# titus-leistner/mmlf

Hardware: AMD Instinct MI355X
Metric: 96x96 EPI patches/sec fwd+bwd, bs=512 (higher is better)
Workload: dtype f32 via 2 x f16 operand split (22 significant bits per operand, locally scaled; 3 MFMA passes, f32 accumulate)

## Files before the change

mmlf_amd/csrc/build.py:

```python
import os
import subprocess
import sys

HERE = os.path.dirname(os.path.abspath(__file__))
SOURCES = ['conv.hip', 'wgrad.hip', 'elementwise.hip']
LIB = os.path.join(HERE, 'libmmlf_hip.so')
HIPCC = os.environ.get('HIPCC', '/opt/rocm/bin/hipcc')
FLAGS = ['-O3', '--offload-arch=gfx950', '-fPIC', '-std=c++17', '-Wall', '-Wno-unused-function', '-ffp-contract=off']


def stale():
    if not os.path.exists(LIB):
        return True
    t = os.path.getmtime(LIB)
    deps = SOURCES + ['common.h', 'conv_device.h', 'build.py', os.path.join('..', '..', 'include', 'mmlf_hip.h')]
    return any(os.path.getmtime(os.path.join(HERE, d)) > t for d in deps)


def source_revision():
    root = os.path.dirname(os.path.dirname(HERE))
    try:
        rev = subprocess.check_output(['git', '-C', root, 'rev-parse', '--short=12', 'HEAD'], stderr=subprocess.DEVNULL).decode().strip()
        dirty = subprocess.call(['git', '-C', root, 'diff', '--quiet', 'HEAD', '--', 'mmlf_amd/csrc', 'include'],
                                stderr=subprocess.DEVNULL) != 0
        return rev + ('+' if dirty else '')
    except (OSError, subprocess.CalledProcessError):
        return 'unknown'


HASHED = SOURCES + ['common.h', 'conv_device.h', os.path.join('..', '..', 'include', 'mmlf_hip.h')]


def source_hash():
    import hashlib
    h = hashlib.sha1()
    for d in HASHED:
        with open(os.path.join(HERE, d), 'rb') as f:
            h.update(f.read())
    return h.hexdigest()[:12]


def build(force=False, verbose=True, extra_flags=(), lib=None):
    if lib is None and not extra_flags and not force and not stale():
        return LIB
    lib = lib or LIB
    tag = '' if lib == LIB else '.' + os.path.basename(lib).replace('.so', '')
    flags = [*FLAGS, f'-DMMLF_GIT_HASH="{source_revision()}"', f'-DMMLF_SRC_HASH="{source_hash()}"', *extra_flags]
    objs, jobs = [], []
    for src in SOURCES:
        obj = os.path.join(os.path.dirname(lib), src.replace('.hip', tag + '.o'))
        cmd = [HIPCC, *flags, '-c', os.path.join(HERE, src), '-o', obj]
        if verbose:
            print(' '.join(cmd), flush=True)
        jobs.append((cmd, subprocess.Popen(cmd)))
        objs.append(obj)
    failed = [cmd for cmd, job in jobs if job.wait() != 0]
    if failed:
        raise subprocess.CalledProcessError(1, failed[0])
    cmd = [HIPCC, '--offload-arch=gfx950', '-shared', '-fPIC', *objs, '-o', lib]
    if verbose:
        print(' '.join(cmd), flush=True)
    subprocess.check_call(cmd)
    return lib


if __name__ == '__main__':
    if '--source-hash' in sys.argv:
        print(source_hash())
    elif '--source-revision' in sys.argv:
        print(source_revision())
    else:
        build(force='--force' in sys.argv)
```

mmlf_amd/csrc/wgrad.hip:

```cpp
#include "conv_device.h"

#ifdef MMLF_BOUNDS_DEBUG
int mmlf_oob_counts_wgrad(unsigned long long *host8, int reset)
{
    if (hipMemcpyFromSymbol(host8, HIP_SYMBOL(g_mmlf_oob), sizeof(unsigned long long) * 8) != hipSuccess) return 1;
    if (reset) {
        const unsigned long long z[8] = {};
        if (hipMemcpyToSymbol(HIP_SYMBOL(g_mmlf_oob), z, sizeof(z)) != hipSuccess) return 1;
    }
    return 0;
}
#endif

struct WgradArgs {
    const float *in;
    const float *g;
    float *part;
    long long NQpad;
    int cs_in, cin, cs_g, g_shift, P, nsplit, nslice, chunks_per_split, nchunks;
    int g_cols;
    const float *in_amax, *g_amax;
    const float *chunk_scales;
    long long in_bytes, g_bytes, part_floats;
};

__device__ __forceinline__ bool wgrad_block_map(const WgradArgs &a, int &slice, int &split)
{
    const int b = blockIdx.x, x = b & 7, j = b >> 3;
    const int reg = (a.nsplit >> 3) * a.nslice;
    if (j < reg) {
        slice = j % a.nslice;
        split = (j / a.nslice) * 8 + x;
        return true;
    }
    const int left = (a.nsplit & 7) * a.nslice, per = (left + 7) >> 3;
    const int m = x * per + (j - reg);
    slice = m % a.nslice;
    split = (a.nsplit & ~7) + m / a.nslice;
    return m < left;
}

static inline unsigned wgrad_grid_blocks(int nslice, int nsplit)
{
    return 8u * (unsigned)((nsplit >> 3) * nslice + ((nsplit & 7) * nslice + 7) / 8);
}

#define WG_KQ 32

template <int KS>
struct WgradF32Shape {
    static constexpr int WAVES = KS == 2 ? 4 : 3;
    static constexpr int SEGS = KS == 2 ? 2 : 1;
    static constexpr int BPS = KS / SEGS;
    static constexpr int ROWS = WG_KQ + KS - 1;
    static constexpr int A_FL = SEGS * ROWS * 32;
    static constexpr size_t lds_bytes(int nt) { return (A_FL + WG_KQ * nt * 32) * sizeof(float); }
};

template <int KS, int NT>
__device__ __forceinline__ void wgrad_f32_taps(const WgradArgs &a)
{
    using S = WgradF32Shape<KS>;
    constexpr int TAPS = KS * KS, THREADS = 64 * S::WAVES, SEGS = S::SEGS, BPS = S::BPS, ROWS = S::ROWS, A_FL = S::A_FL;
    constexpr int NP = NT * 32;
    constexpr int A_F4 = A_FL / 4;
    constexpr int NA = (A_F4 + THREADS - 1) / THREADS;
    constexpr int G_F4 = WG_KQ * NP / 4;
    constexpr int NG = (G_F4 + THREADS - 1) / THREADS;
    static_assert(KS == 3 || G_F4 % THREADS == 0, "2x2: the gradient tile is a whole number of staging rounds (no guard)");
    extern __shared__ __attribute__((aligned(16))) char smem[];
    float *As = reinterpret_cast<float *>(smem);
    float *Gs = As + A_FL;

    const int tid = threadIdx.x;
    const int lane = tid & 63, wv = tid >> 6;
    const int i = lane & 31, kh = lane >> 5;
    int sd, split;
    if (!wgrad_block_map(a, sd, split)) return;
    const int slice = sd / BPS, dy = sd - BPS * slice;
    const int ci0 = slice * 32;
    int c_begin = split * a.chunks_per_split;
    int c_end = c_begin + a.chunks_per_split;
    if (c_end > a.nchunks) c_end = a.nchunks;

    f32x16 acc[NT];
#pragma unroll
    for (int nt = 0; nt < NT; ++nt)
#pragma unroll
        for (int r = 0; r < 16; ++r) acc[nt][r] = 0.f;

    float4 ra[NA], rg[NG];
    auto gload = [&](int c) {
        const long long Qc = (long long)c * WG_KQ + (long long)dy * a.P;
#pragma unroll
        for (int j = 0; j < NA; ++j) {
            const int idx = tid + THREADS * j;
            float4 v = make_float4(0.f, 0.f, 0.f, 0.f);
            if (idx < A_F4) {
                const int row = idx >> 3, f = idx & 7;
                const int seg = SEGS > 1 && row >= ROWS, pix = row - ROWS * seg;
                const int ch = ci0 + 4 * f;
                if (ch < a.cs_in)
                    v = *reinterpret_cast<const float4 *>(a.in + (size_t)(Qc + seg * a.P + pix) * a.cs_in + ch);
            }
            ra[j] = v;
        }
        const long long Qg = (long long)c * WG_KQ + a.g_shift;
#pragma unroll
        for (int j = 0; j < NG; ++j) {
            const int idx = tid + THREADS * j;
            float4 v = make_float4(0.f, 0.f, 0.f, 0.f);
            if (KS == 2 || idx < G_F4) {
                const int row = idx / (NP / 4), f = idx - row * (NP / 4);
                if (4 * f < a.g_cols) v = *reinterpret_cast<const float4 *>(a.g + (size_t)(Qg + row) * a.cs_g + 4 * f);
            }
            rg[j] = v;
        }
    };
    auto lstore = [&]() {
#pragma unroll
        for (int j = 0; j < NA; ++j) {
            const int idx = tid + THREADS * j;
            if (idx < A_F4) {
                float4 v = ra[j];
                const int ch = ci0 + 4 * (idx & 7);
                if (ch == a.cin) v.x = 1.f;
                if (ch + 1 == a.cin) v.y = 1.f;
                if (ch + 2 == a.cin) v.z = 1.f;
                if (ch + 3 == a.cin) v.w = 1.f;
                reinterpret_cast<float4 *>(As)[idx] = v;
            }
        }
#pragma unroll
        for (int j = 0; j < NG; ++j) {
            const int idx = tid + THREADS * j;
            if (KS == 2 || idx < G_F4) reinterpret_cast<float4 *>(Gs)[idx] = rg[j];
        }
    };

    const int seg = KS == 2 ? wv >> 1 : 0, dx = KS == 2 ? wv & 1 : wv;
    if (c_begin < c_end) {
        gload(c_begin);
        for (int c = c_begin; c < c_end; ++c) {
            lstore();
            __syncthreads();
            if (c + 1 < c_end) gload(c + 1);
            const float *ap = As + (seg * ROWS + dx + kh) * 32 + i;
            const float *gp = Gs + kh * NP + i;
#pragma unroll
            for (int s = 0; s < WG_KQ / 2; ++s) {
                const float av = ap[2 * s * 32];
#pragma unroll
                for (int nt = 0; nt < NT; ++nt) {
                    const float bv = gp[2 * s * NP + 32 * nt];
                    acc[nt] = __builtin_amdgcn_mfma_f32_32x32x2f32(av, bv, acc[nt], 0, 0, 0);
                }
            }
            __syncthreads();
        }
    }
    const int CIP = a.nslice / BPS * 32;
    float *pp = a.part + ((size_t)(split * TAPS + KS * (dy + seg) + dx) * CIP + ci0) * NP;
#pragma unroll
    for (int nt = 0; nt < NT; ++nt)
#pragma unroll
        for (int r = 0; r < 16; ++r) {
            const int row = (r & 3) + 8 * (r >> 2) + 4 * kh;
            pp[(size_t)row * NP + 32 * nt + i] = acc[nt][r];
        }
}

template <int NT>
__global__ __launch_bounds__(256, 2) void wgrad4tap_kernel(WgradArgs a)
{
    wgrad_f32_taps<2, NT>(a);
}

template <int NT>
__global__ __launch_bounds__(192, 2) void wgrad9tap_kernel(WgradArgs a)
{
    wgrad_f32_taps<3, NT>(a);
}

typedef short s16x4 __attribute__((ext_vector_type(4)));
typedef __attribute__((address_space(3))) s16x4 lds_s16x4_t;

__device__ __forceinline__ bf16x8 tr_frag(const char *lds_row0, int row_stride_bytes)
{
    const s16x4 lo = __builtin_amdgcn_ds_read_tr16_b64_v4i16((lds_s16x4_t *)(lds_row0));
    const s16x4 hi = __builtin_amdgcn_ds_read_tr16_b64_v4i16((lds_s16x4_t *)(lds_row0 + 4 * row_stride_bytes));
    return __builtin_shufflevector(lo, hi, 0, 1, 2, 3, 4, 5, 6, 7);
}

__device__ __forceinline__ void split_store4(float4 v, char *p0, int plane_stride_bytes)
{
    unsigned h0, m0, l0, h1, m1, l1;
    split3_pair(v.x, v.y, h0, m0, l0);
    split3_pair(v.z, v.w, h1, m1, l1);
    *reinterpret_cast<uint2 *>(p0) = make_uint2(h0, h1);
    *reinterpret_cast<uint2 *>(p0 + plane_stride_bytes) = make_uint2(m0, m1);
    *reinterpret_cast<uint2 *>(p0 + 2 * plane_stride_bytes) = make_uint2(l0, l1);
}

template <int PL>
__device__ __forceinline__ void split_store4_pl(float4 v, float scale, char *p0, int plane_stride_bytes)
{
    if constexpr (PL == 3) {
        split_store4(v, p0, plane_stride_bytes);
    } else {
        unsigned h0, l0, h1, l1;
        split2_pair_f16<true>(v.x, v.y, scale, h0, l0);
        split2_pair_f16<true>(v.z, v.w, scale, h1, l1);
        *reinterpret_cast<uint2 *>(p0) = make_uint2(h0, h1);
        *reinterpret_cast<uint2 *>(p0 + plane_stride_bytes) = make_uint2(l0, l1);
    }
}
template <int PL>
__device__ __forceinline__ f32x4 mfma16_pl(bf16x8 x, bf16x8 y, f32x4 c)
{
    if constexpr (PL == 3) return __builtin_amdgcn_mfma_f32_16x16x32_bf16(x, y, c, 0, 0, 0);
    else return __builtin_amdgcn_mfma_f32_16x16x32_f16(__builtin_bit_cast(f16x8, x), __builtin_bit_cast(f16x8, y), c, 0, 0, 0);
}
template <int PL> __device__ __forceinline__ constexpr int term_a(int t)
{
    return PL == 3 ? (t == 0 ? 2 : t == 1 ? 0 : t <= 3 ? 1 : 0) : (t == 0 ? 1 : 0);
}
template <int PL> __device__ __forceinline__ constexpr int term_b(int t)
{
    return PL == 3 ? (t == 0 ? 0 : t == 1 ? 2 : t == 2 ? 1 : t == 3 ? 0 : t == 4 ? 1 : 0) : (t == 1 ? 1 : 0);
}
struct WgradScales { float inv_sa, inv_sg; };
template <int PL> __device__ __forceinline__ WgradScales wgrad_scales(const WgradArgs &a)
{
    WgradScales s = {1.f, 1.f};
    if constexpr (PL == 2) {
        s.inv_sa = a.chunk_scales[2 * (size_t)a.nchunks];
        s.inv_sg = a.chunk_scales[2 * (size_t)a.nchunks + 1];
    }
    return s;
}
template <int PL> __device__ __forceinline__ void wgrad_chunk_scale(const WgradArgs &a, int c, float &sa, float &sg)
{
    if constexpr (PL == 2) {
        const float2 v = *reinterpret_cast<const float2 *>(a.chunk_scales + 2 * (size_t)c);
        sa = __uint_as_float(__builtin_amdgcn_readfirstlane(__float_as_uint(v.x)));
        sg = __uint_as_float(__builtin_amdgcn_readfirstlane(__float_as_uint(v.y)));
    } else {
        sa = 1.f; sg = 1.f;
    }
}
struct ChunkScaleArgs {
    const float *in_amax, *g_amax;
    float *out;
    long long NQ;
    int nchunks, P, g_shift, nrows;
    Magic divP;
};
__device__ __forceinline__ int pow2_exponent(float p) { return (int)(__float_as_uint(p) >> 23) - 127; }
__global__ __launch_bounds__(256) void wgrad_chunk_scales_kernel(ChunkScaleArgs a)
{
    const int c = blockIdx.x * 256 + threadIdx.x;
    const float sA = pow2_scale_for(mmlf_amax_tensor_max(a.in_amax)), sG = pow2_scale_for(mmlf_amax_tensor_max(a.g_amax));
    if (c == 0) {
        a.out[2 * (size_t)a.nchunks] = 1.f / sA;
        a.out[2 * (size_t)a.nchunks + 1] = 1.f / sG;
    }
    if (c >= a.nchunks) return;
    const long long q0 = (long long)c * WG_KQ;
    int x = 0;
    if (q0 < a.NQ) {
        const long long ql = q0 + WG_KQ - 1;
        const unsigned r0 = fastdiv((unsigned)q0, a.divP);
        unsigned r1 = fastdiv((unsigned)(ql + a.P + 1), a.divP);
        if (r1 >= (unsigned)a.nrows) r1 = a.nrows - 1;
        float ma = 0.f, mg = 0.f;
        for (unsigned r = r0; r <= r1; ++r) ma = fmaxf(ma, a.in_amax[MMLF_AMAX_HEAD + r]);
        const unsigned g0 = fastdiv((unsigned)(q0 + a.g_shift), a.divP);
        unsigned g1 = fastdiv((unsigned)(ql + a.g_shift), a.divP);
        if (g1 >= (unsigned)a.nrows) g1 = a.nrows - 1;
        for (unsigned r = g0; r <= g1; ++r) mg = fmaxf(mg, a.g_amax[MMLF_AMAX_HEAD + r]);
        const int u = ma > 0.f ? pow2_exponent(pow2_scale_for(ma)) - pow2_exponent(sA) : 60;
        const int v = mg > 0.f ? pow2_exponent(pow2_scale_for(mg)) - pow2_exponent(sG) : 60;
        const int uu = u < 0 ? 0 : u, vv = v < 0 ? 0 : v;
        x = (uu - vv) >> 1;
        x = x > 15 ? 15 : (x < -24 ? -24 : x);
    }
    a.out[2 * (size_t)c] = sA * exp2f((float)x);
    a.out[2 * (size_t)c + 1] = sG * exp2f((float)-x);
}

template <int MB, int NB, int PL>
__global__ __launch_bounds__(256, 2) void wgrad4tap_x6n_kernel(WgradArgs a)
{
    constexpr int ROWA = 32 * (MB | 1), ROWG = 32 * (NB | 1);
    constexpr int A_PLANE = 34 * ROWA;
    constexpr int A_BYTES = 2 * PL * A_PLANE;
    constexpr int NTERM = PL == 3 ? 6 : 3;
    const WgradScales sc = wgrad_scales<PL>(a);
    constexpr int G_PLANE = WG_KQ * ROWG;
    constexpr int FA = 4 * MB, FG = 4 * NB;
    constexpr int NA = (66 * FA + 255) / 256, NG = (WG_KQ * FG + 255) / 256;
    constexpr bool HOLD_G = NB <= 5;
    extern __shared__ __attribute__((aligned(16))) char smem[];
    char *As = smem;
    char *Gs = smem + A_BYTES;

    const int tid = threadIdx.x;
    const int lane = tid & 63, t = tid >> 6;
    const int r16 = lane & 15, q4 = lane >> 4;
    int slice, split;
    if (!wgrad_block_map(a, slice, split)) return;
    const int ci0 = slice * 16 * MB;
    int c_begin = split * a.chunks_per_split;
    int c_end = c_begin + a.chunks_per_split;
    if (c_end > a.nchunks) c_end = a.nchunks;

    f32x4 acc[MB][NB];
#pragma unroll
    for (int mb = 0; mb < MB; ++mb)
#pragma unroll
        for (int nb = 0; nb < NB; ++nb)
#pragma unroll
            for (int r = 0; r < 4; ++r) acc[mb][nb][r] = 0.f;

    float4 ra[NA], rg[NG];
#define WN_GLOAD(c)                                                                                         \
    do {                                                                                                    \
        const long long Qc = (long long)(c) * WG_KQ;                                                        \
        _Pragma("unroll") for (int j = 0; j < NA; ++j) {                                                    \
            const int idx = min(tid + 256 * j, 66 * FA - 1);                                                \
            const int row = idx / FA, f = idx - row * FA;                                                   \
            const int seg = row >= 33, pix = row - 33 * seg;                                                \
            const int ch = min(ci0 + 4 * f, a.cs_in - 4);                                                   \
            MMLF_OOB(OOB_WG_IN, ((Qc + seg * a.P + pix) * a.cs_in + ch + 4) * 4ll > a.in_bytes);            \
            ra[j] = *reinterpret_cast<const float4 *>(a.in + (size_t)(Qc + seg * a.P + pix) * a.cs_in + ch); \
        }                                                                                                   \
        _Pragma("unroll") for (int j = 0; j < NG; ++j) {                                                    \
            const int idx = min(tid + 256 * j, WG_KQ * FG - 1);                                             \
            const int row = idx / FG, f = idx - row * FG;                                                   \
            const int gc = min(4 * f, a.g_cols - 4);                                                        \
            MMLF_OOB(OOB_WG_G, ((Qc + a.g_shift + row) * a.cs_g + gc + 4) * 4ll > a.g_bytes);               \
            rg[j] = *reinterpret_cast<const float4 *>(a.g + (size_t)(Qc + a.g_shift + row) * a.cs_g + gc);  \
        }                                                                                                   \
    } while (0)
#define WN_LSTORE()                                                                                         \
    do {                                                                                                    \
        _Pragma("unroll") for (int j = 0; j < NA; ++j) {                                                    \
            const int idx = min(tid + 256 * j, 66 * FA - 1);                                                \
            const int row = idx / FA, f = idx - row * FA;                                                   \
            const int seg = row >= 33, pix = row - 33 * seg;                                                \
            float4 v = ra[j];                \
            const int ch = ci0 + 4 * f;      \
            if (ch == a.cin) v.x = sc.inv_sa;                                        \
            if (ch + 1 == a.cin) v.y = sc.inv_sa;                                                           \
            if (ch + 2 == a.cin) v.z = sc.inv_sa;                                                           \
            if (ch + 3 == a.cin) v.w = sc.inv_sa;                                                           \
            split_store4_pl<PL>(v, st_sa, As + seg * PL * A_PLANE + pix * ROWA + 8 * f, A_PLANE);           \
        }                                                                                                   \
        _Pragma("unroll") for (int j = 0; j < NG; ++j) {                                                    \
            const int idx = min(tid + 256 * j, WG_KQ * FG - 1);                                             \
            const int row = idx / FG, f = idx - row * FG;                                                   \
            split_store4_pl<PL>(rg[j], st_sg, Gs + row * ROWG + 8 * f, G_PLANE);                            \
        }                                                                                                   \
    } while (0)
    const int tq = (lane & 15) >> 2, tp = lane & 3;
    const char *a_lane = As + (t >> 1) * PL * A_PLANE + ((t & 1) + 4 * q4 + tq) * ROWA + 8 * tp;
    const char *g_lane = Gs + (4 * q4 + tq) * ROWG + 8 * tp;

    float st_sa = 1.f, st_sg = 1.f;
    if (c_begin < c_end) {
        WN_GLOAD(c_begin);
        for (int c = c_begin; c < c_end; ++c) {
            wgrad_chunk_scale<PL>(a, c, st_sa, st_sg);
            WN_LSTORE();
            __syncthreads();
            if (c + 1 < c_end) WN_GLOAD(c + 1);
            if constexpr (HOLD_G) {
                bf16x8 gf[NB][PL];
#pragma unroll
                for (int nb = 0; nb < NB; ++nb)
#pragma unroll
                    for (int pl = 0; pl < PL; ++pl) gf[nb][pl] = tr_frag(g_lane + pl * G_PLANE + 32 * nb, 4 * ROWG);
#pragma unroll
                for (int mb = 0; mb < MB; ++mb) {
                    bf16x8 af[PL];
#pragma unroll
                    for (int pl = 0; pl < PL; ++pl) af[pl] = tr_frag(a_lane + pl * A_PLANE + 32 * mb, 4 * ROWA);
#pragma unroll
                    for (int term = 0; term < NTERM; ++term)
#pragma unroll
                        for (int nb = 0; nb < NB; ++nb)
                            acc[mb][nb] = mfma16_pl<PL>(af[term_a<PL>(term)], gf[nb][term_b<PL>(term)], acc[mb][nb]);
                }
            } else {
                bf16x8 af[MB][PL];
#pragma unroll
                for (int mb = 0; mb < MB; ++mb)
#pragma unroll
                    for (int pl = 0; pl < PL; ++pl) af[mb][pl] = tr_frag(a_lane + pl * A_PLANE + 32 * mb, 4 * ROWA);
#pragma unroll
                for (int nb = 0; nb < NB; ++nb) {
                    bf16x8 gf[PL];
#pragma unroll
                    for (int pl = 0; pl < PL; ++pl) gf[pl] = tr_frag(g_lane + pl * G_PLANE + 32 * nb, 4 * ROWG);
#pragma unroll
                    for (int term = 0; term < NTERM; ++term)
#pragma unroll
                        for (int mb = 0; mb < MB; ++mb)
                            acc[mb][nb] = mfma16_pl<PL>(af[mb][term_a<PL>(term)], gf[term_b<PL>(term)], acc[mb][nb]);
                }
            }
            __syncthreads();
        }
    }
#undef WN_GLOAD
#undef WN_LSTORE
    constexpr int NP = 16 * NB;
    const int CIP = a.nslice * 16 * MB;
    float *pp = a.part + ((size_t)(split * 4 + t) * CIP + ci0) * NP;
#pragma unroll
    for (int mb = 0; mb < MB; ++mb)
#pragma unroll
        for (int nb = 0; nb < NB; ++nb)
#pragma unroll
            for (int r = 0; r < 4; ++r) {
                const int row = 16 * mb + 4 * q4 + r;
                const float un = (ci0 + row == a.cin ? 1.f : sc.inv_sa) * sc.inv_sg;
                MMLF_OOB(OOB_WG_PART, (long long)(pp - a.part) + (long long)row * NP + 16 * nb + r16 >= a.part_floats);
                pp[(size_t)row * NP + 16 * nb + r16] = acc[mb][nb][r] * un;
            }
}

template <int MB, int NBH, int PL>
__global__ __launch_bounds__(512, 2) void wgrad4tap_x6w_kernel(WgradArgs a)
{
    constexpr int NB = 2 * NBH;
    const WgradScales sc = wgrad_scales<PL>(a);
    constexpr int ROWA = 32 * (MB | 1), ROWG = 32 * (NB | 1);
    constexpr int A_PLANE = 34 * ROWA;
    constexpr int A_BYTES = 2 * PL * A_PLANE;
    constexpr int G_PLANE = WG_KQ * ROWG;
    constexpr int BUF_BYTES = A_BYTES + PL * G_PLANE;
    constexpr int FA = 4 * MB, FG = 4 * NB;
    constexpr int NA = (66 * FA + 511) / 512, NG = (WG_KQ * FG + 511) / 512;
    static_assert(2 * BUF_BYTES <= 160 * 1024, "LDS");
    extern __shared__ __attribute__((aligned(16))) char smem[];

    const int tid = threadIdx.x;
    const int lane = tid & 63;
    const int w = __builtin_amdgcn_readfirstlane(tid >> 6);
    const int t = w & 3, h = w >> 2;
    const int r16 = lane & 15, q4 = lane >> 4;
    int slice, split;
    if (!wgrad_block_map(a, slice, split)) return;
    const int ci0 = slice * 16 * MB;
    const int c_begin = split * a.chunks_per_split;
    int c_end = c_begin + a.chunks_per_split;
    if (c_end > a.nchunks) c_end = a.nchunks;

    f32x4 acc[MB][NBH];
#pragma unroll
    for (int mb = 0; mb < MB; ++mb)
#pragma unroll
        for (int nb = 0; nb < NBH; ++nb)
#pragma unroll
            for (int r = 0; r < 4; ++r) acc[mb][nb][r] = 0.f;

    float4 ra[NA], rg[NG];

    unsigned ga_off[NA], gg_off[NG];
    int la_off[NA], lg_off[NG], a_ch[NA];
#pragma unroll
    for (int j = 0; j < NA; ++j) {
        const int idx = min(tid + 512 * j, 66 * FA - 1);
        const int row = idx / FA, f = idx - row * FA;
        const int seg = row >= 33, pix = row - 33 * seg;
        a_ch[j] = ci0 + 4 * f;
        ga_off[j] = (unsigned)((seg * a.P + pix) * a.cs_in + min(ci0 + 4 * f, a.cs_in - 4)) * 4u;
        la_off[j] = seg * PL * A_PLANE + pix * ROWA + 8 * f;
    }
#pragma unroll
    for (int j = 0; j < NG; ++j) {
        const int idx = min(tid + 512 * j, WG_KQ * FG - 1);
        const int row = idx / FG, f = idx - row * FG;
        gg_off[j] = (unsigned)((a.g_shift + row) * a.cs_g + min(4 * f, a.g_cols - 4)) * 4u;
        lg_off[j] = A_BYTES + row * ROWG + 8 * f;
    }
    const char *const in_b = reinterpret_cast<const char *>(a.in), *const g_b = reinterpret_cast<const char *>(a.g);
#define WW_GLOAD_A(j, c)                                                                                    \
    do {                                                                                                    \
        const long long cb_ = (long long)(c) * WG_KQ * a.cs_in * 4;                         \
        MMLF_OOB(OOB_WG_IN, cb_ + ga_off[j] + 16 > a.in_bytes);                                             \
         \
         \
        const __amdgpu_buffer_rsrc_t rs_ = __builtin_amdgcn_make_buffer_rsrc(                               \
            const_cast<char *>(in_b + cb_), 0, mmlf_records_left(a.in_bytes, cb_), MMLF_BUF_FLAGS);         \
        ra[j] = __builtin_bit_cast(float4, __builtin_amdgcn_raw_buffer_load_b128(rs_, ga_off[j], 0, 0));    \
    } while (0)
#define WW_GLOAD_G(j, c)                                                                                    \
    do {                                                                                                    \
        const long long cb_ = (long long)(c) * WG_KQ * a.cs_g * 4;                                          \
        MMLF_OOB(OOB_WG_G, cb_ + gg_off[j] + 16 > a.g_bytes);                                               \
        const __amdgpu_buffer_rsrc_t rs_ = __builtin_amdgcn_make_buffer_rsrc(                               \
            const_cast<char *>(g_b + cb_), 0, mmlf_records_left(a.g_bytes, cb_), MMLF_BUF_FLAGS);           \
        rg[j] = __builtin_bit_cast(float4, __builtin_amdgcn_raw_buffer_load_b128(rs_, gg_off[j], 0, 0));    \
    } while (0)
#define WW_GLOAD(c)                                                                                         \
    do {                                                                                                    \
        _Pragma("unroll") for (int j = 0; j < NA; ++j) WW_GLOAD_A(j, c);                                    \
        _Pragma("unroll") for (int j = 0; j < NG; ++j) WW_GLOAD_G(j, c);                                    \
    } while (0)
#define WW_STORE_A(j, dst)                                                                                  \
    do {                                                                                                    \
        float4 v = ra[j];                                                    \
        const int ch = a_ch[j];                                                                             \
        v.x = ch == a.cin ? sc.inv_sa : v.x;                                         \
        v.y = ch + 1 == a.cin ? sc.inv_sa : v.y;                                                            \
        v.z = ch + 2 == a.cin ? sc.inv_sa : v.z;                                                            \
        v.w = ch + 3 == a.cin ? sc.inv_sa : v.w;                                                            \
        split_store4_pl<PL>(v, st_sa, (dst) + la_off[j], A_PLANE);                                          \
    } while (0)
#define WW_STORE_G(j, dst) split_store4_pl<PL>(rg[j], st_sg, (dst) + lg_off[j], G_PLANE)

    const int tq = (lane & 15) >> 2, tp = lane & 3;
    const int a_off = (t >> 1) * PL * A_PLANE + ((t & 1) + 4 * q4 + tq) * ROWA + 8 * tp;
    const int g_off = A_BYTES + (4 * q4 + tq) * ROWG + 8 * tp + 32 * NBH * h;

    float st_sa = 1.f, st_sg = 1.f;
    if (c_begin < c_end) {
        WW_GLOAD(c_begin);
        wgrad_chunk_scale<PL>(a, c_begin, st_sa, st_sg);
#pragma unroll
        for (int j = 0; j < NA; ++j) WW_STORE_A(j, smem);
#pragma unroll
        for (int j = 0; j < NG; ++j) WW_STORE_G(j, smem);
        if (c_begin + 1 < c_end) WW_GLOAD(c_begin + 1);
        __syncthreads();
        int buf = 0;
        constexpr bool EARLY = PL == 2 && NBH % 3 == 0 && NA + NG <= NBH - 2 && MB >= 2;
        bf16x8 af[MB][PL], gfr[3][PL], afp[2][PL];
        if constexpr (EARLY) {
            const char *cur0 = smem;
#pragma unroll
            for (int g0 = 0; g0 < 2; ++g0)
#pragma unroll
                for (int pl = 0; pl < PL; ++pl) gfr[g0][pl] = tr_frag(cur0 + g_off + pl * G_PLANE + 32 * g0, 4 * ROWG);
#pragma unroll
            for (int mb = 0; mb < 2; ++mb)
#pragma unroll
                for (int pl = 0; pl < PL; ++pl) af[mb][pl] = tr_frag(cur0 + a_off + pl * A_PLANE + 32 * mb, 4 * ROWA);
        }
#define WW_TERM(gf, pa, pb)                                                                                  \
    _Pragma("unroll") for (int mb = 0; mb < MB; ++mb)                                                        \
        acc[mb][nb] = mfma16_pl<PL>(af[mb][pa], gf[pb], acc[mb][nb])
#define WW_CHUNK(STAGE, RELOAD)                                                                              \
    do {                                                                                                     \
        const char *cur = smem + buf * BUF_BYTES;                                                            \
        char *nxt = smem + (buf ^ 1) * BUF_BYTES;                                                            \
        if (!EARLY) {                                                                                        \
            _Pragma("unroll") for (int g0 = 0; g0 < 2; ++g0)                                                 \
                _Pragma("unroll") for (int pl = 0; pl < PL; ++pl)                                             \
                    gfr[g0][pl] = tr_frag(cur + g_off + pl * G_PLANE + 32 * g0, 4 * ROWG);                   \
        }                                                                                                    \
        _Pragma("unroll") for (int mb = EARLY ? 2 : 0; mb < MB; ++mb)                                        \
            _Pragma("unroll") for (int pl = 0; pl < PL; ++pl)                                                 \
                af[mb][pl] = tr_frag(cur + a_off + pl * A_PLANE + 32 * mb, 4 * ROWA);                        \
        _Pragma("unroll") for (int nb = 0; nb < NBH; ++nb) {                                                 \
            if (EARLY && (STAGE) && nb == NBH - 2) {                                                         \
                asm volatile("s_waitcnt lgkmcnt(0)" ::: "memory");    \
                __syncthreads();                                                                             \
                _Pragma("unroll") for (int mb = 0; mb < 2; ++mb)                                             \
                    _Pragma("unroll") for (int pl = 0; pl < PL; ++pl)                                         \
                        afp[mb][pl] = tr_frag(nxt + a_off + pl * A_PLANE + 32 * mb, 4 * ROWA);               \
            }                                                                                                \
            if (nb + 2 < NBH) {                                                                              \
                _Pragma("unroll") for (int pl = 0; pl < PL; ++pl)                                             \
                    gfr[(nb + 2) % 3][pl] = tr_frag(cur + g_off + pl * G_PLANE + 32 * (nb + 2), 4 * ROWG);   \
            } else if (EARLY && (STAGE)) {                                                                   \
                _Pragma("unroll") for (int pl = 0; pl < PL; ++pl)                                             \
                    gfr[(nb + 2) % 3][pl] = tr_frag(nxt + g_off + pl * G_PLANE + 32 * (nb + 2 - NBH), 4 * ROWG); \
            }                                                                                                \
            if (STAGE) {                                                                                     \
                if (nb < NA) {                                                                               \
                    WW_STORE_A(nb < NA ? nb : 0, nxt);                                                       \
                    if (RELOAD) WW_GLOAD_A(nb < NA ? nb : 0, c + 2);                                         \
                } else if (nb - NA < NG) {                                                                   \
                    WW_STORE_G(nb - NA < NG ? nb - NA : 0, nxt);                                             \
                    if (RELOAD) WW_GLOAD_G(nb - NA < NG ? nb - NA : 0, c + 2);                               \
                }                                                                                            \
            }                                                                                                \
            _Pragma("unroll") for (int term = 0; term < (PL == 3 ? 6 : 3); ++term)                           \
                WW_TERM(gfr[nb % 3], term_a<PL>(term), term_b<PL>(term));                                    \
        }                                                                                                    \
        if (EARLY && (STAGE)) {                                                                              \
            _Pragma("unroll") for (int mb = 0; mb < 2; ++mb)                                                 \
                _Pragma("unroll") for (int pl = 0; pl < PL; ++pl) af[mb][pl] = afp[mb][pl];                   \
        }                                                                                                    \
    } while (0)
        static_assert(NA + NG <= NBH, "one staging piece per column block");
        for (int c = c_begin; c + 1 < c_end; ++c) {
            wgrad_chunk_scale<PL>(a, c + 1, st_sa, st_sg);
            const bool reload = c + 2 < c_end;
            WW_CHUNK(true, reload);
            if constexpr (!EARLY) __syncthreads();
            buf ^= 1;
        }
        {
            const int c = c_end - 1;
            (void)c;
            WW_CHUNK(false, false);
        }
#undef WW_CHUNK
#undef WW_TERM
    }
#undef WW_GLOAD
#undef WW_GLOAD_A
#undef WW_GLOAD_G
#undef WW_STORE_A
#undef WW_STORE_G
    constexpr int NP = 16 * NB;
    const int CIP = a.nslice * 16 * MB;
    float *pp = a.part + ((size_t)(split * 4 + t) * CIP + ci0) * NP + 16 * NBH * h;
#pragma unroll
    for (int mb = 0; mb < MB; ++mb)
#pragma unroll
        for (int nb = 0; nb < NBH; ++nb)
#pragma unroll
            for (int r = 0; r < 4; ++r) {
                const int row = 16 * mb + 4 * q4 + r;
                const float un = (ci0 + row == a.cin ? 1.f : sc.inv_sa) * sc.inv_sg;
                MMLF_OOB(OOB_WG_PART, (long long)(pp - a.part) + (long long)row * NP + 16 * nb + r16 >= a.part_floats);
                pp[(size_t)row * NP + 16 * nb + r16] = acc[mb][nb][r] * un;
            }
}

template <int NTAP>
__global__ void wgrad_reduce_kernel(const float *__restrict__ part, float *__restrict__ gw, float *__restrict__ gb,
                                     int Cin, int Cout, int CIP, int NP, int nsplit, int variant, int accumulate)
{
    const int total = NTAP * (Cin + 1) * Cout;
    const int idx = blockIdx.x * blockDim.x + threadIdx.x;
    if (idx >= total) return;
    const int co = idx % Cout;
    int r = idx / Cout;
    const int ci = r % (Cin + 1);
    const int t = r / (Cin + 1);
    if (ci == Cin && (t != 0 || gb == nullptr)) return;
    const float *pp = part + ((size_t)t * CIP + ci) * NP + co;
    const size_t stride = (size_t)NTAP * CIP * NP;
    constexpr int U = 16;
    double acc[U];
#pragma unroll
    for (int u = 0; u < U; ++u) acc[u] = 0.0;
    int sp = 0;
    for (; sp + U <= nsplit; sp += U) {
        float v[U];
#pragma unroll
        for (int u = 0; u < U; ++u) v[u] = pp[(size_t)(sp + u) * stride];
#pragma unroll
        for (int u = 0; u < U; ++u) acc[u] += v[u];
    }
    for (; sp < nsplit; ++sp) acc[0] += pp[(size_t)sp * stride];
#pragma unroll
    for (int h = U / 2; h > 0; h >>= 1)
#pragma unroll
        for (int u = 0; u < h; ++u) acc[u] += acc[u + h];
    const double s = acc[0];
    if (ci == Cin) {
        gb[co] = accumulate ? gb[co] + (float)s : (float)s;
    } else {
        const size_t o = ((size_t)co * Cin + ci) * NTAP + master_tap<(NTAP == 4 ? 2 : 3)>(t, variant);
        gw[o] = accumulate ? gw[o] + (float)s : (float)s;
    }
}

__global__ __launch_bounds__(256) void wgrad_reduce_wave_kernel(const float *__restrict__ part, float *__restrict__ gw,
                                                                float *__restrict__ gb, int Cin, int Cout, int CIP, int NP,
                                                                int nsplit, int variant, int accumulate)
{
    const int total = 4 * (Cin + 1) * Cout;
    const int idx = blockIdx.x * 4 + (threadIdx.x >> 6), lane = threadIdx.x & 63;
    if (idx >= total) return;
    const int co = idx % Cout;
    int r = idx / Cout;
    const int ci = r % (Cin + 1);
    const int t = r / (Cin + 1);
    if (ci == Cin && (t != 0 || gb == nullptr)) return;
    const float *pp = part + ((size_t)t * CIP + ci) * NP + co;
    const size_t stride = (size_t)4 * CIP * NP;
    double acc = 0.0;
    for (int sp = lane; sp < nsplit; sp += 64) acc += pp[(size_t)sp * stride];
#pragma unroll
    for (int o = 32; o > 0; o >>= 1) acc += __shfl_xor(acc, o);
    if (lane) return;
    if (ci == Cin) {
        gb[co] = accumulate ? gb[co] + (float)acc : (float)acc;
    } else {
        const size_t o = ((size_t)co * Cin + ci) * 4 + master_tap<2>(t, variant);
        gw[o] = accumulate ? gw[o] + (float)acc : (float)acc;
    }
}

static int wgrad_nsplit(int nslice)
{
    int n = 512 / nslice;
    n = n / 8 * 8;
    if (n < 8) n = 8;
    return n;
}

struct Wgrad16Cfg { int mb, nb, nslice, nsplit; };
static inline bool wgrad16_cfg(int Cin, int Cout, long long nchunks, Wgrad16Cfg *c)
{
    if (Cout <= 0 || Cout > 288) return false;
    c->nb = Cout <= 32 ? 2 : Cout <= 80 ? 5 : Cout <= 128 ? 8 : 18;
    if (c->nb == 18) {
        c->mb = 3;
        c->nslice = (Cin + 1 + 47) / 48;
        const int cus = nchunks < 0 ? 256 : (device_cus() < 256 ? device_cus() : 256);
        const int one_round = cus / c->nslice, three_rounds = (768 / c->nslice + 7) / 8 * 8;
        c->nsplit = nchunks < 0 ? (one_round > three_rounds ? one_round : three_rounds)
                                : (nchunks >= 42 * 1024 ? three_rounds : one_round);
        if (c->nsplit < 8) c->nsplit = 8;
    } else {
        c->mb = (c->nb <= 5 && Cin + 1 > 32 && Cin + 1 <= 80) ? 5 : 2;
        if (c->nb == 8 && Cin + 1 >= 128) c->mb = 3;
        c->nslice = (Cin + 1 + 16 * c->mb - 1) / (16 * c->mb);
        c->nsplit = wgrad_nsplit(c->nslice);
    }
    return true;
}

constexpr int WGRAD_MAX_COUT = 288, WGRAD_MAX_COUT_WIDE = 512;
static inline int wgrad_col_blocks(int Cout) { return Cout > WGRAD_MAX_COUT ? 2 : 1; }
static inline int wgrad_block_cout(int Cout, int b) { return b == 0 ? (Cout < WGRAD_MAX_COUT ? Cout : WGRAD_MAX_COUT) : Cout - WGRAD_MAX_COUT; }

struct WgradBlock {
    int c0, cout;
    int nt;
    Wgrad16Cfg cfg;
    int nslice, nsplit;
    int CIP, NP;
    int64_t part_floats;
};
struct WgradPlan {
    int nblocks;
    WgradBlock blk[2];
    int64_t part_floats;
    int64_t scales_off;
};
static bool wgrad_f32_block(int ks, int Cin, int c0, int cout, WgradBlock &k)
{
    k = {};
    k.c0 = c0; k.cout = cout; k.nt = pick_nt(cout);
    if (k.nt < 0) return false;
    const int ci_slices = (Cin + 1 + 31) / 32;
    k.nslice = (ks == 2 ? WgradF32Shape<2>::BPS : WgradF32Shape<3>::BPS) * ci_slices;
    k.nsplit = wgrad_nsplit(k.nslice);
    k.CIP = ci_slices * 32; k.NP = k.nt * 32;
    k.part_floats = (int64_t)k.nsplit * ks * ks * k.CIP * k.NP;
    return true;
}
static void wgrad_split_block(const Wgrad16Cfg &c, WgradBlock &k)
{
    k.nt = 0; k.cfg = c; k.nslice = c.nslice; k.nsplit = c.nsplit;
    k.CIP = c.nslice * 16 * c.mb; k.NP = 16 * c.nb;
    k.part_floats = (int64_t)k.nsplit * 4 * k.CIP * k.NP;
}
static bool wgrad_plan(int planes, int Cin, int Cout, long long nchunks, WgradPlan &p)
{
    p = {};
    if (Cout > WGRAD_MAX_COUT_WIDE) return false;
    p.nblocks = wgrad_col_blocks(Cout);
    for (int b = 0, c0 = 0; b < p.nblocks; c0 += p.blk[b++].cout) {
        WgradBlock &k = p.blk[b];
        WgradBlock largest = {};
        Wgrad16Cfg c;
        if (!wgrad_f32_block(2, Cin, c0, wgrad_block_cout(Cout, b), k)) return false;
        int64_t sized = k.part_floats;
        if (wgrad16_cfg(Cin, k.cout, -1, &c)) {
            wgrad_split_block(c, largest);
            if (largest.part_floats > sized) sized = largest.part_floats;
        }
        sized = (sized + 3) / 4 * 4;
        if (sized > p.scales_off) p.scales_off = sized;
        if (planes && wgrad16_cfg(Cin, k.cout, nchunks, &c)) wgrad_split_block(c, k);
        if (k.part_floats > p.part_floats) p.part_floats = k.part_floats;
    }
    return true;
}

extern "C" int64_t mmlf_wgrad_workspace_floats(int Cin, int Cout, int B, int H, int W)
{
    WgradPlan p;
    if (!wgrad_plan(0, Cin, Cout, -1, p) || B <= 0 || H <= 0 || W <= 0) return -1;
    return p.scales_off + 2 * (make_grid(B, H, W).NQpad / WG_KQ) + 4;
}

template <int KS, int NT>
static int launch_wgrad_f32(const WgradArgs &a, hipStream_t st)
{
    using S = WgradF32Shape<KS>;
    const dim3 grid(wgrad_grid_blocks(a.nslice, a.nsplit)), block(64 * S::WAVES);
    if constexpr (KS == 2) hipLaunchKernelGGL(wgrad4tap_kernel<NT>, grid, block, S::lds_bytes(NT), st, a);
    else hipLaunchKernelGGL(wgrad9tap_kernel<NT>, grid, block, S::lds_bytes(NT), st, a);
    return mmlf_launch_status(KS == 2 ? "mmlf_conv2x2_wgrad" : "mmlf_conv3x3_wgrad");
}

template <int MB, int NB, int PL>
static int launch_wgrad16(const WgradArgs &a, hipStream_t st)
{
    constexpr size_t lds = 2 * PL * 34 * 32 * (MB | 1) + PL * WG_KQ * 32 * (NB | 1);
    static PerDeviceOnce attr_once;
    if (attr_once.run([] { return mmlf_allow_lds(reinterpret_cast<const void *>(wgrad4tap_x6n_kernel<MB, NB, PL>), lds, "mmlf_conv2x2_wgrad_split"); }))
        return 1;
    hipLaunchKernelGGL((wgrad4tap_x6n_kernel<MB, NB, PL>), dim3(wgrad_grid_blocks(a.nslice, a.nsplit)), dim3(256), lds, st, a);
    return mmlf_launch_status("mmlf_conv2x2_wgrad_split");
}

template <int PL>
static int launch_wgrad_wide(const WgradArgs &a, hipStream_t st)
{
    constexpr size_t lds = 2 * (2 * PL * 34 * 32 * (3 | 1) + PL * WG_KQ * 32 * (18 | 1));
    static PerDeviceOnce attr_once;
    if (attr_once.run([] { return mmlf_allow_lds(reinterpret_cast<const void *>(wgrad4tap_x6w_kernel<3, 9, PL>), lds, "mmlf_conv2x2_wgrad_split(wide)"); }))
        return 1;
    hipLaunchKernelGGL((wgrad4tap_x6w_kernel<3, 9, PL>), dim3(wgrad_grid_blocks(a.nslice, a.nsplit)), dim3(512), lds, st, a);
    return mmlf_launch_status("mmlf_conv2x2_wgrad_split");
}

template <int PL>
static int launch_wgrad_split(const Wgrad16Cfg &c, const WgradArgs &a, hipStream_t st)
{
    switch (10 * c.mb + c.nb) {
    case 22: return launch_wgrad16<2, 2, PL>(a, st);
    case 52: return launch_wgrad16<5, 2, PL>(a, st);
    case 25: return launch_wgrad16<2, 5, PL>(a, st);
    case 55: return launch_wgrad16<5, 5, PL>(a, st);
    case 28: return launch_wgrad16<2, 8, PL>(a, st);
    case 38: return launch_wgrad16<3, 8, PL>(a, st);
    default: return launch_wgrad_wide<PL>(a, st);
    }
}

static WgradArgs wgrad_args(const float *in, int cs_in, int Cin, const float *g, int cs_g, int g_shift, float *workspace,
                            const Grid &gr, long long alloc, long long part_floats)
{
    WgradArgs a = {};
    a.in = in; a.g = g; a.part = workspace; a.NQpad = gr.NQpad;
    a.cs_in = cs_in; a.cin = Cin; a.cs_g = a.g_cols = cs_g; a.g_shift = g_shift; a.P = gr.P;
    a.in_bytes = alloc * cs_in * 4; a.g_bytes = alloc * cs_g * 4;
    a.part_floats = part_floats;
    a.nchunks = (int)(gr.NQpad / WG_KQ);
    return a;
}
static void wgrad_set_grid(WgradArgs &a, int nslice, int nsplit)
{
    a.nslice = nslice;
    a.nsplit = nsplit;
    a.chunks_per_split = (a.nchunks + nsplit - 1) / nsplit;
}

template <int KS>
static int wgrad_reduce(const WgradArgs &a, float *gw, float *gb, int Cin, int Cout, int CIP, int NP, int variant,
                        int accumulate, hipStream_t st)
{
    const int total = KS * KS * (Cin + 1) * Cout;
    hipLaunchKernelGGL(wgrad_reduce_kernel<KS * KS>, dim3((total + 255) / 256), dim3(256), 0, st, a.part, gw, gb, Cin, Cout,
                       CIP, NP, a.nsplit, variant, accumulate);
    return mmlf_launch_status(KS == 2 ? "mmlf_conv2x2_wgrad(reduce)" : "mmlf_conv3x3_wgrad(reduce)");
}

template <int KS>
static int wgrad_run_block(WgradArgs &a, const WgradBlock &k, int planes, float *gw, float *gb, int Cin, int variant,
                           int accumulate, hipStream_t st)
{
    wgrad_set_grid(a, k.nslice, k.nsplit);
    int rc = 1;
    if constexpr (KS == 2) {
        if (!k.nt) rc = planes == 3 ? launch_wgrad_split<3>(k.cfg, a, st) : launch_wgrad_split<2>(k.cfg, a, st);
    }
    if (k.nt) switch (k.nt) {
    case 1: rc = launch_wgrad_f32<KS, 1>(a, st); break;
    case 3: rc = launch_wgrad_f32<KS, 3>(a, st); break;
    case 4: rc = launch_wgrad_f32<KS, 4>(a, st); break;
    default: rc = launch_wgrad_f32<KS, 9>(a, st); break;
    }
    if (rc) return rc;
    return wgrad_reduce<KS>(a, gw, gb, Cin, k.cout, k.CIP, k.NP, variant, accumulate, st);
}

static int wgrad_impl(const float *in, int cs_in, int Cin, const float *g, int cs_g, int Cout, int g_shift,
                      float *gw, float *gb, int variant, int accumulate, float *workspace, int B, int H, int W,
                      void *stream, int planes, const float *in_amax = nullptr, const float *g_amax = nullptr);

extern "C" int mmlf_conv2x2_wgrad(const float *in, int cs_in, int Cin, const float *g, int cs_g, int Cout,
                                  int g_shift, float *gw, float *gb, int variant, int accumulate,
                                  float *workspace, int B, int H, int W, void *stream)
{
    return wgrad_impl(in, cs_in, Cin, g, cs_g, Cout, g_shift, gw, gb, variant, accumulate, workspace, B, H, W,
                      stream, 0);
}

extern "C" int mmlf_conv2x2_wgrad_split(const float *in, int cs_in, int Cin, const float *g, int cs_g, int Cout,
                                        int g_shift, float *gw, float *gb, int variant, int accumulate,
                                        float *workspace, int B, int H, int W, void *stream)
{
    return wgrad_impl(in, cs_in, Cin, g, cs_g, Cout, g_shift, gw, gb, variant, accumulate, workspace, B, H, W,
                      stream, 3);
}

extern "C" int mmlf_conv2x2_wgrad_h2(const float *in, int cs_in, int Cin, const float *g, int cs_g, int Cout,
                                     int g_shift, float *gw, float *gb, int variant, int accumulate,
                                     float *workspace, int B, int H, int W, const float *in_amax,
                                     const float *g_amax, void *stream)
{
    MMLF_CHECK_ARG(in_amax && g_amax, "mmlf_conv2x2_wgrad_h2: the f16 split needs max |in| and max |g|");
    return wgrad_impl(in, cs_in, Cin, g, cs_g, Cout, g_shift, gw, gb, variant, accumulate, workspace, B, H, W,
                      stream, 2, in_amax, g_amax);
}

static int wgrad_impl(const float *in, int cs_in, int Cin, const float *g, int cs_g, int Cout, int g_shift,
                      float *gw, float *gb, int variant, int accumulate, float *workspace, int B, int H, int W,
                      void *stream, int planes, const float *in_amax, const float *g_amax)
{
    MMLF_CHECK_ARG(in && g && gw && workspace, "mmlf_conv2x2_wgrad: null pointer");
    MMLF_CHECK_ARG(cs_in % 4 == 0 && cs_g % 4 == 0, "mmlf_conv2x2_wgrad: strides must be multiples of 4");
    MMLF_CHECK_ARG(Cin > 0 && Cin <= cs_in && Cout > 0 && Cout <= cs_g, "mmlf_conv2x2_wgrad: channels vs strides");
    MMLF_CHECK_ARG(Cout <= WGRAD_MAX_COUT_WIDE, "mmlf_conv2x2_wgrad: Cout=%d not supported (max %d)", Cout, WGRAD_MAX_COUT_WIDE);
    MMLF_CHECK_ARG(variant >= 0 && variant <= 2, "mmlf_conv2x2_wgrad: bad variant");
    Grid gr = make_grid(B, H, W);
    MMLF_CHECK_ARG(g_shift >= 0 && g_shift <= gr.P + 1, "mmlf_conv2x2_wgrad: g_shift=%d", g_shift);
    WgradPlan p;
    MMLF_CHECK_ARG(wgrad_plan(planes, Cin, Cout, gr.NQpad / WG_KQ, p), "mmlf_conv2x2_wgrad: no launch plan");
    WgradArgs a = wgrad_args(in, cs_in, Cin, g, cs_g, g_shift, workspace, gr, grid_alloc_positions(gr), p.scales_off);
    a.in_amax = in_amax; a.g_amax = g_amax;
    hipStream_t st = (hipStream_t)stream;
    if (planes == 2) {
        MMLF_CHECK_ARG(gr.NQpad + 2 * gr.P + 64 < (1ll << 31), "mmlf_conv2x2_wgrad_h2: batch x image too large");
        ChunkScaleArgs ca;
        ca.in_amax = in_amax; ca.g_amax = g_amax; ca.out = workspace + p.scales_off;
        ca.NQ = gr.NQ; ca.nchunks = a.nchunks; ca.P = gr.P; ca.g_shift = g_shift;
        ca.nrows = (int)amax_rows(gr);
        ca.divP = make_magic((unsigned)gr.P);
        hipLaunchKernelGGL(wgrad_chunk_scales_kernel, dim3((a.nchunks + 255) / 256), dim3(256), 0, st, ca);
        a.chunk_scales = ca.out;
    }
    const WgradArgs whole = a;
    for (int b = 0; b < p.nblocks; ++b) {
        const int c0 = p.blk[b].c0;
        a = whole;
        a.g = g + c0; a.g_cols = cs_g - c0; a.g_bytes = whole.g_bytes - 4ll * c0;
        const int rc = wgrad_run_block<2>(a, p.blk[b], planes, gw + (size_t)c0 * Cin * 4, gb ? gb + c0 : nullptr, Cin, variant,
                                          accumulate, st);
        if (rc) return rc;
    }
    return 0;
}

__global__ __launch_bounds__(256) void thin_wgrad_kernel(ThinArgs a)
{
    const int lane = threadIdx.x & 63;
    const long long wave = __builtin_amdgcn_readfirstlane((int)(blockIdx.x * 4 + (threadIdx.x >> 6)));
    const long long nwaves = gridDim.x * 4ll;
    float acc[2][4][THIN_MAXN][4];
#pragma unroll
    for (int h = 0; h < 2; ++h)
#pragma unroll
        for (int t = 0; t < 4; ++t)
#pragma unroll
            for (int o = 0; o < THIN_MAXN; ++o)
#pragma unroll
                for (int k = 0; k < 4; ++k) acc[h][t][o][k] = 0.f;
    float gsum[THIN_MAXN] = {0.f, 0.f};
    const bool first = 4 * lane < a.cs_in, second = 256 + 4 * lane < a.cs_in;
    const int offs[4] = {0, 1, a.P, a.P + 1};
    constexpr int U = 4;
    for (long long p0 = U * wave; p0 < a.npos; p0 += U * nwaves) {
        float4 x0[U], x1[U];
        float gt[U][4][THIN_MAXN];
#pragma unroll
        for (int u = 0; u < U; ++u) {
            const long long p = p0 + u < a.npos ? p0 + u : a.npos - 1;
            const float *row = a.in + (size_t)p * a.cs_in;
            x0[u] = first ? *reinterpret_cast<const float4 *>(row + 4 * lane) : make_float4(0.f, 0.f, 0.f, 0.f);
            x1[u] = second ? *reinterpret_cast<const float4 *>(row + 256 + 4 * lane) : make_float4(0.f, 0.f, 0.f, 0.f);
#pragma unroll
            for (int t = 0; t < 4; ++t) {
                const long long q = p0 + u - offs[t];
                const bool ok = p0 + u < a.npos && q >= 0 && q < a.NQ;
                const float2 gv = *reinterpret_cast<const float2 *>(a.g + (size_t)((ok ? q : 0) + a.g_shift) * a.cs_g);
                gt[u][t][0] = ok ? gv.x : 0.f;
                gt[u][t][1] = ok ? gv.y : 0.f;
            }
        }
#pragma unroll
        for (int u = 0; u < U; ++u) {
            const float xs[2][4] = {{x0[u].x, x0[u].y, x0[u].z, x0[u].w}, {x1[u].x, x1[u].y, x1[u].z, x1[u].w}};
#pragma unroll
            for (int h = 0; h < 2; ++h)
#pragma unroll
                for (int t = 0; t < 4; ++t)
#pragma unroll
                    for (int o = 0; o < THIN_MAXN; ++o)
#pragma unroll
                        for (int k = 0; k < 4; ++k) acc[h][t][o][k] = fmaf(xs[h][k], gt[u][t][o], acc[h][t][o][k]);
#pragma unroll
            for (int o = 0; o < THIN_MAXN; ++o) gsum[o] += gt[u][0][o];
        }
    }
    float *pp = a.wpart + (size_t)wave * 4 * a.CIP * THIN_MAXN;
#pragma unroll
    for (int h = 0; h < 2; ++h)
// ... 108 lines not shown
```

Measured before the change: 1149.

## Make wide 2x2 wgrad kernel persistent with a grid-stride loop over work items

The wide wgrad kernel now loops over (slice, split) work items with a grid-stride loop, and the launch is capped at the number of resident CUs (rounded down to a multiple of 8). Per-item state, including accumulators, global offsets and the partial-sum store, moves inside the loop. The aim is to avoid a tail of partially filled waves when the item count exceeds one round of CUs. In exchange it adds an extra __syncthreads per item and risks load imbalance, since items are assigned statically rather than dynamically scheduled. The block-mapping helpers move into a shared header, and an env var can turn persistence off.

```diff
diff --git a/mmlf_amd/csrc/build.py b/mmlf_amd/csrc/build.py
--- a/mmlf_amd/csrc/build.py
+++ b/mmlf_amd/csrc/build.py
@@ -13,7 +13,7 @@
     if not os.path.exists(LIB):
         return True
     t = os.path.getmtime(LIB)
-    deps = SOURCES + ['common.h', 'conv_device.h', 'build.py', os.path.join('..', '..', 'include', 'mmlf_hip.h')]
+    deps = SOURCES + ['common.h', 'conv_device.h', 'wgrad_map.h', 'build.py', os.path.join('..', '..', 'include', 'mmlf_hip.h')]
     return any(os.path.getmtime(os.path.join(HERE, d)) > t for d in deps)
 
 
@@ -28,7 +28,7 @@
         return 'unknown'
 
 
-HASHED = SOURCES + ['common.h', 'conv_device.h', os.path.join('..', '..', 'include', 'mmlf_hip.h')]
+HASHED = SOURCES + ['common.h', 'conv_device.h', 'wgrad_map.h', os.path.join('..', '..', 'include', 'mmlf_hip.h')]
 
 
 def source_hash():
diff --git a/mmlf_amd/csrc/wgrad.hip b/mmlf_amd/csrc/wgrad.hip
--- a/mmlf_amd/csrc/wgrad.hip
+++ b/mmlf_amd/csrc/wgrad.hip
@@ -1,4 +1,5 @@
 #include "conv_device.h"
+#include "wgrad_map.h"
 
 #ifdef MMLF_BOUNDS_DEBUG
 int mmlf_oob_counts_wgrad(unsigned long long *host8, int reset)
@@ -18,32 +19,12 @@
     float *part;
     long long NQpad;
     int cs_in, cin, cs_g, g_shift, P, nsplit, nslice, chunks_per_split, nchunks;
+    int items;
     int g_cols;
     const float *in_amax, *g_amax;
     const float *chunk_scales;
     long long in_bytes, g_bytes, part_floats;
 };
-
-__device__ __forceinline__ bool wgrad_block_map(const WgradArgs &a, int &slice, int &split)
-{
-    const int b = blockIdx.x, x = b & 7, j = b >> 3;
-    const int reg = (a.nsplit >> 3) * a.nslice;
-    if (j < reg) {
-        slice = j % a.nslice;
-        split = (j / a.nslice) * 8 + x;
-        return true;
-    }
-    const int left = (a.nsplit & 7) * a.nslice, per = (left + 7) >> 3;
-    const int m = x * per + (j - reg);
-    slice = m % a.nslice;
-    split = (a.nsplit & ~7) + m / a.nslice;
-    return m < left;
-}
-
-static inline unsigned wgrad_grid_blocks(int nslice, int nsplit)
-{
-    return 8u * (unsigned)((nsplit >> 3) * nslice + ((nsplit & 7) * nslice + 7) / 8);
-}
 
 #define WG_KQ 32
 
@@ -76,7 +57,7 @@
     const int lane = tid & 63, wv = tid >> 6;
     const int i = lane & 31, kh = lane >> 5;
     int sd, split;
-    if (!wgrad_block_map(a, sd, split)) return;
+    if (!wgrad_block_map(blockIdx.x, a.nslice, a.nsplit, sd, split)) return;
     const int slice = sd / BPS, dy = sd - BPS * slice;
     const int ci0 = slice * 32;
     int c_begin = split * a.chunks_per_split;
@@ -309,7 +290,7 @@
     const int lane = tid & 63, t = tid >> 6;
     const int r16 = lane & 15, q4 = lane >> 4;
     int slice, split;
-    if (!wgrad_block_map(a, slice, split)) return;
+    if (!wgrad_block_map(blockIdx.x, a.nslice, a.nsplit, slice, split)) return;
     const int ci0 = slice * 16 * MB;
     int c_begin = split * a.chunks_per_split;
     int c_end = c_begin + a.chunks_per_split;
@@ -450,21 +431,7 @@
     const int lane = tid & 63;
     const int w = __builtin_amdgcn_readfirstlane(tid >> 6);
     const int t = w & 3, h = w >> 2;
-    const int r16 = lane & 15, q4 = lane >> 4;
-    int slice, split;
-    if (!wgrad_block_map(a, slice, split)) return;
-    const int ci0 = slice * 16 * MB;
-    const int c_begin = split * a.chunks_per_split;
-    int c_end = c_begin + a.chunks_per_split;
-    if (c_end > a.nchunks) c_end = a.nchunks;
-
-    f32x4 acc[MB][NBH];
-#pragma unroll
-    for (int mb = 0; mb < MB; ++mb)
-#pragma unroll
-        for (int nb = 0; nb < NBH; ++nb)
-#pragma unroll
-            for (int r = 0; r < 4; ++r) acc[mb][nb][r] = 0.f;
+    const int q4 = lane >> 4;
 
     float4 ra[NA], rg[NG];
 
@@ -475,8 +442,6 @@
         const int idx = min(tid + 512 * j, 66 * FA - 1);
         const int row = idx / FA, f = idx - row * FA;
         const int seg = row >= 33, pix = row - 33 * seg;
-        a_ch[j] = ci0 + 4 * f;
-        ga_off[j] = (unsigned)((seg * a.P + pix) * a.cs_in + min(ci0 + 4 * f, a.cs_in - 4)) * 4u;
         la_off[j] = seg * PL * A_PLANE + pix * ROWA + 8 * f;
     }
 #pragma unroll
@@ -523,12 +488,45 @@
 #define WW_STORE_G(j, dst) split_store4_pl<PL>(rg[j], st_sg, (dst) + lg_off[j], G_PLANE)
 
     const int tq = (lane & 15) >> 2, tp = lane & 3;
-    const int a_off = (t >> 1) * PL * A_PLANE + ((t & 1) + 4 * q4 + tq) * ROWA + 8 * tp;
-    const int g_off = A_BYTES + (4 * q4 + tq) * ROWG + 8 * tp + 32 * NBH * h;
+    int a_off = (t >> 1) * PL * A_PLANE + ((t & 1) + 4 * q4 + tq) * ROWA + 8 * tp;
+    int g_off = A_BYTES + (4 * q4 + tq) * ROWG + 8 * tp + 32 * NBH * h;
+
+    for (int b = blockIdx.x; b < a.items; b += gridDim.x) {
+    int slice, split;
+    if (!wgrad_block_map(b, a.nslice, a.nsplit, slice, split)) continue;
+    const int ci0 = slice * 16 * MB;
+    const int c_begin = split * a.chunks_per_split;
+    int c_end = c_begin + a.chunks_per_split;
+    if (c_end > a.nchunks) c_end = a.nchunks;
+
+    f32x4 acc[MB][NBH];
+#pragma unroll
+    for (int mb = 0; mb < MB; ++mb)
+#pragma unroll
+        for (int nb = 0; nb < NBH; ++nb)
+#pragma unroll
+            for (int r = 0; r < 4; ++r) acc[mb][nb][r] = 0.f;
+#pragma unroll
+    for (int j = 0; j < NA; ++j) asm volatile("" : "+v"(la_off[j]));
+#pragma unroll
+    for (int j = 0; j < NG; ++j) asm volatile("" : "+v"(lg_off[j]), "+v"(gg_off[j]));
+    asm volatile("" : "+v"(a_off), "+v"(g_off));
+    int tid_i;
+    asm volatile("v_mbcnt_lo_u32_b32 %0, -1, 0\n\tv_mbcnt_hi_u32_b32 %0, -1, %0" : "=v"(tid_i));
+    tid_i += 64 * w;
+#pragma unroll
+    for (int j = 0; j < NA; ++j) {
+        const int idx = min(tid_i + 512 * j, 66 * FA - 1);
+        const int row = idx / FA, f = idx - row * FA;
+        const int seg = row >= 33, pix = row - 33 * seg;
+        a_ch[j] = ci0 + 4 * f;
+        ga_off[j] = (unsigned)((seg * a.P + pix) * a.cs_in + min(ci0 + 4 * f, a.cs_in - 4)) * 4u;
+    }
 
     float st_sa = 1.f, st_sg = 1.f;
     if (c_begin < c_end) {
         WW_GLOAD(c_begin);
+        __syncthreads();
         wgrad_chunk_scale<PL>(a, c_begin, st_sa, st_sg);
 #pragma unroll
         for (int j = 0; j < NA; ++j) WW_STORE_A(j, smem);
@@ -610,28 +608,32 @@
             (void)c;
             WW_CHUNK(false, false);
         }
+    }
+    constexpr int NP = 16 * NB;
+    const int CIP = a.nslice * 16 * MB;
+    float *pp = a.part + ((size_t)(split * 4 + t) * CIP + ci0) * NP + 16 * NBH * h;
+    int tid_e;
+    asm volatile("v_mbcnt_lo_u32_b32 %0, -1, 0\n\tv_mbcnt_hi_u32_b32 %0, -1, %0" : "=v"(tid_e));
+    const int r16e = tid_e & 15, q4e = (tid_e & 63) >> 4;
+#pragma unroll
+    for (int mb = 0; mb < MB; ++mb)
+#pragma unroll
+        for (int nb = 0; nb < NBH; ++nb)
+#pragma unroll
+            for (int r = 0; r < 4; ++r) {
+                const int row = 16 * mb + 4 * q4e + r;
+                const float un = (ci0 + row == a.cin ? 1.f : sc.inv_sa) * sc.inv_sg;
+                MMLF_OOB(OOB_WG_PART, (long long)(pp - a.part) + (long long)row * NP + 16 * nb + r16e >= a.part_floats);
+                pp[(size_t)row * NP + 16 * nb + r16e] = acc[mb][nb][r] * un;
+            }
+    }
 #undef WW_CHUNK
 #undef WW_TERM
-    }
 #undef WW_GLOAD
 #undef WW_GLOAD_A
 #undef WW_GLOAD_G
 #undef WW_STORE_A
 #undef WW_STORE_G
-    constexpr int NP = 16 * NB;
-    const int CIP = a.nslice * 16 * MB;
-    float *pp = a.part + ((size_t)(split * 4 + t) * CIP + ci0) * NP + 16 * NBH * h;
-#pragma unroll
-    for (int mb = 0; mb < MB; ++mb)
-#pragma unroll
-        for (int nb = 0; nb < NBH; ++nb)
-#pragma unroll
-            for (int r = 0; r < 4; ++r) {
-                const int row = 16 * mb + 4 * q4 + r;
-                const float un = (ci0 + row == a.cin ? 1.f : sc.inv_sa) * sc.inv_sg;
-                MMLF_OOB(OOB_WG_PART, (long long)(pp - a.part) + (long long)row * NP + 16 * nb + r16 >= a.part_floats);
-                pp[(size_t)row * NP + 16 * nb + r16] = acc[mb][nb][r] * un;
-            }
 }
 
 template <int NTAP>
@@ -716,12 +718,7 @@
     c->nb = Cout <= 32 ? 2 : Cout <= 80 ? 5 : Cout <= 128 ? 8 : 18;
     if (c->nb == 18) {
         c->mb = 3;
-        c->nslice = (Cin + 1 + 47) / 48;
-        const int cus = nchunks < 0 ? 256 : (device_cus() < 256 ? device_cus() : 256);
-        const int one_round = cus / c->nslice, three_rounds = (768 / c->nslice + 7) / 8 * 8;
-        c->nsplit = nchunks < 0 ? (one_round > three_rounds ? one_round : three_rounds)
-                                : (nchunks >= 42 * 1024 ? three_rounds : one_round);
-        if (c->nsplit < 8) c->nsplit = 8;
+        wgrad_wide_splits(Cin, nchunks, device_cus(), c->nslice, c->nsplit);
     } else {
         c->mb = (c->nb <= 5 && Cin + 1 > 32 && Cin + 1 <= 80) ? 5 : 2;
         if (c->nb == 8 && Cin + 1 >= 128) c->mb = 3;
@@ -818,6 +815,12 @@
     return mmlf_launch_status("mmlf_conv2x2_wgrad_split");
 }
 
+static bool wgrad_persist()
+{
+    static const bool on = [] { const char *e = getenv("MMLF_WGRAD_PERSIST"); return !e || atoi(e) != 0; }();
+    return on;
+}
+
 template <int PL>
 static int launch_wgrad_wide(const WgradArgs &a, hipStream_t st)
 {
@@ -825,7 +828,7 @@
     static PerDeviceOnce attr_once;
     if (attr_once.run([] { return mmlf_allow_lds(reinterpret_cast<const void *>(wgrad4tap_x6w_kernel<3, 9, PL>), lds, "mmlf_conv2x2_wgrad_split(wide)"); }))
         return 1;
-    hipLaunchKernelGGL((wgrad4tap_x6w_kernel<3, 9, PL>), dim3(wgrad_grid_blocks(a.nslice, a.nsplit)), dim3(512), lds, st, a);
+    hipLaunchKernelGGL((wgrad4tap_x6w_kernel<3, 9, PL>), dim3(wgrad_wide_grid(a.items, device_cus(), wgrad_persist())), dim3(512), lds, st, a);
     return mmlf_launch_status("mmlf_conv2x2_wgrad_split");
 }
 
@@ -859,6 +862,7 @@
     a.nslice = nslice;
     a.nsplit = nsplit;
     a.chunks_per_split = (a.nchunks + nsplit - 1) / nsplit;
+    a.items = (int)wgrad_grid_blocks(nslice, nsplit);
 }
 
 template <int KS>
diff --git a/mmlf_amd/csrc/wgrad_map.h b/mmlf_amd/csrc/wgrad_map.h
--- /dev/null
+++ b/mmlf_amd/csrc/wgrad_map.h
@@ -0,0 +1,40 @@
+#pragma once
+
+__host__ __device__ __forceinline__ bool wgrad_block_map(int b, int nslice, int nsplit, int &slice, int &split)
+{
+    const int x = b & 7, j = b >> 3;
+    const int reg = (nsplit >> 3) * nslice;
+    if (j < reg) {
+        slice = j % nslice;
+        split = (j / nslice) * 8 + x;
+        return true;
+    }
+    const int left = (nsplit & 7) * nslice, per = (left + 7) >> 3;
+    const int m = x * per + (j - reg);
+    slice = m % nslice;
+    split = (nsplit & ~7) + m / nslice;
+    return m < left;
+}
+
+static inline unsigned wgrad_grid_blocks(int nslice, int nsplit)
+{
+    return 8u * (unsigned)((nsplit >> 3) * nslice + ((nsplit & 7) * nslice + 7) / 8);
+}
+
+static inline void wgrad_wide_splits(int Cin, long long nchunks, int cus, int &nslice, int &nsplit)
+{
+    nslice = (Cin + 1 + 47) / 48;
+    if (cus > 256 || nchunks < 0) cus = 256;
+    const int one_round = cus / nslice, three_rounds = (768 / nslice + 7) / 8 * 8;
+    nsplit = nchunks < 0 ? (one_round > three_rounds ? one_round : three_rounds)
+                         : (nchunks >= 42 * 1024 ? three_rounds : one_round);
+    if (nsplit < 8) nsplit = 8;
+}
+
+static inline unsigned wgrad_wide_grid(int items, int cus, bool persist)
+{
+    if (!persist) return (unsigned)items;
+    int resident = cus / 8 * 8;
+    if (resident < 8) resident = 8;
+    return (unsigned)(items < resident ? items : resident);
+}
```

New measurement: 1163 (median of 6 runs). +1.2%, better.
